# google-research/frame-interpolation

Measured on NVIDIA H100. Metric: interpolated_frames_per_sec_1080p, higher is better.
Workload: dtype f16x2-split (activations/weights as fp16 hi+lo planes; fp32 accumulate)

## Files before the change

frame_interpolation_b200/csrc/film_conv.h:

```cpp
#pragma once
#include <cuda.h>
#include <stdint.h>

#include "film_common.cuh"

namespace film {

constexpr int kMaxSrc = 4;
constexpr int kMaxTaps = 9;
constexpr int kChunk = 64;
constexpr int kTileM = 128;

struct ConvSrc {
  const sp_t* hi;
  const sp_t* lo;
  int C;
  int c_off;
  int nchunk;
  int bswap;
};

struct alignas(64) ConvProblem {
  CUtensorMap tm_a_hi[kMaxSrc];
  CUtensorMap tm_a_lo[kMaxSrc];
// ... 25 lines not shown
  const float* head_b3;
  int crop_y, crop_x, crop_h, crop_w;
  int64_t crop_pitch;
  const float* head_w4;
  const float* head_b4;
  const float* head_vup;
  float* head_res;
  float* head_v;
  int v2_resident;
  int v2_na, v2_nw;
  int v2_grid;
  int v2_part_lo, v2_part_hi;
  sp_t* pool_hi;
  sp_t* pool_lo;
  int pool_C;
  int group;
  int pair;
  int halo;
  int bn;
  int passes;
  int straight;
  int out_lo_skip;
  int pxn;
};

cudaError_t launch_conv_tc(const ConvProblem* d_prob, const ConvProblem& h_prob, cudaStream_t st);
cudaError_t launch_conv_simt(const ConvProblem* d_prob, const ConvProblem& h_prob, cudaStream_t st);
cudaError_t conv_tc_configure();
bool conv3x3_tc_plan(ConvProblem& h_prob, int num_sms);
void conv3x3_tc_pick_tile(int H, int W, int B, int cout, int kc, int passes, int ktot, int epi_mode, int num_sms,
                          int& tile_h, int& tile_w);
cudaError_t launch_conv3x3_tc(const ConvProblem* d_prob, const ConvProblem& h_prob, cudaStream_t st);
cudaError_t conv3x3_tc_configure();
}
```

frame_interpolation_b200/csrc/film_conv3x3_tc.cu:

```cuda
#include <cuda.h>
#include <cuda_runtime.h>
#include <stdint.h>

#include <type_traits>

#include "film_conv.h"
#include "film_tc_ptx.cuh"

namespace film {
namespace {
using namespace tc;

constexpr int kConsumers = 256;
constexpr int kThreads = kConsumers + 128;
__host__ __device__ constexpr int a_plane_bytes(int kc, int th, int tw) { return (th + 2) * tw * kc * 2; }
__host__ __device__ constexpr int a_stage_bytes(int kc, int th, int tw) { return 2 * a_plane_bytes(kc, th, tw); }
constexpr int kHaloW = 10;
__host__ __device__ constexpr int halo_box_bytes(int kc, int th) { return (th + 2) * kHaloW * kc * 2; }
__host__ __device__ constexpr int halo_plane_bytes(int kc, int th) { return (halo_box_bytes(kc, th) + 1023) & ~1023; }
__host__ __device__ constexpr int a_stage_bytes_h(int kc, int th, int tw, int halo, int planes = 2) {
  return planes * (halo ? halo_plane_bytes(kc, th) : a_plane_bytes(kc, th, tw));
}
constexpr int kMaxRing = 8;
constexpr int kSmemLimit = 227 * 1024;
constexpr int kBarBytes = 8 * (4 * kMaxRing + 4);
constexpr int kFixedBytes = kBarBytes + 16 + 512 * 4  + 64  + 1024  + 64;
constexpr int kHeadW3 = 64 * 32 * 4, kHeadMisc = 512;
constexpr int kHeadBytes = kHeadW3 + kHeadMisc;
constexpr int kPxnStageWg = 64 * 64 * 2;
constexpr int kPxnStageBytes = 2 * kPxnStageWg;
inline int epi_scratch_bytes(int epi_mode, int pxn) { return epi_mode == 3 ? kHeadBytes : pxn ? kPxnStageBytes : 0; }

__host__ __device__ inline int w_tap_bytes(int bn, int kc, int planes = 2) { return bn * kc * 2 * planes; }

template <int BN, int KC, bool kPartial, bool kHalo, bool kOne, bool kRes, bool kPxN = false>
__global__ void __launch_bounds__(kThreads, 1) k_conv3x3_tc(const ConvProblem* __restrict__ prob) {
  static_assert(!kPxN || (BN == 64 && KC == 64), "pixels on N: Cout = 64 (one M = 64 weight tile), 64-channel chunks");
  extern __shared__ uint8_t smem_raw[];
  constexpr bool one = kOne;
  const int planes = one ? 1 : 2;
  constexpr int kWPlane = BN * KC * 2;
  const int kWTap = kWPlane * planes;
  const int kTileH = prob->tile_h, kTileW = prob->tile_w;
  constexpr int kHaloTileH = kPxN ? 32 : 16;
  constexpr int kHaloBox = halo_box_bytes(KC, kHaloTileH), kHaloPlane = halo_plane_bytes(KC, kHaloTileH);
  constexpr bool halo = kHalo;
  const int kAPlane = halo ? kHaloPlane : a_plane_bytes(KC, kTileH, kTileW);
  const int kAStage = planes * kAPlane;
  const int kRowStep = kTileW * KC * 2;
  constexpr bool kFused = BN <= 128 && !kPxN;
  constexpr int kAccRegs = kPxN ? 64 : (kFused ? 2 * BN : BN) / 2;
  constexpr int kWgPx = kPxN ? 128 : 64;

  const int NA = prob->v2_na, NW = prob->v2_nw;
  const bool resident = prob->v2_resident != 0;
  const int nsrc = prob->nsrc;
  const int tiles_x = prob->tiles_x, tiles_per_img = prob->tiles_y * prob->tiles_x;
  const int cout = prob->cout;
  const int n_nt = (cout + BN - 1) / BN;
  const int ntiles = prob->B * tiles_per_img * n_nt;
  constexpr int kStageTaps = kHalo ? 9 : 3;
  constexpr bool kPacked = kPartial && kPxN;
  const int part_lo = prob->v2_part_lo, part_hi = prob->v2_part_hi;
  int nab = 0;
// ... 72 lines not shown
      {
        const int nt = tile + w_step;
        int next_sp, nnt;
        decode(nt < nwork ? nt : 0, next_sp, nnt);
        if (nt < nwork && next_sp != sp && next_sp < nsp && elect_one()) {
          int nb, nrem, nty, ntx;
          div_img.divmod(next_sp, nb, nrem);
          div_tx.divmod(nrem, nty, ntx);
          const int ny0 = nty * kTileH, nx0 = ntx * kTileW;
          for (int s = 0; s < nsrc; ++s)
            for (int ch = 0; ch < src_tab[2 * s]; ++ch) {
              const int cc = src_tab[2 * s + 1] + ch * KC;
              tma_prefetch_4d(&prob->tm_a_hi[s], cc, nx0 - 1, ny0 - 1, nb);
              if (!one) tma_prefetch_4d(&prob->tm_a_lo[s], cc, nx0 - 1, ny0 - 1, nb);
              if (!halo) {
                tma_prefetch_4d(&prob->tm_a_hi[s], cc, nx0 + 1, ny0 - 1, nb);
                if (!one) tma_prefetch_4d(&prob->tm_a_lo[s], cc, nx0 + 1, ny0 - 1, nb);
              }
            }
        }
        __syncwarp();
      }
      int kb = 0, ab = 0;
      for (int s = 0; s < nsrc; ++s) {
        const int nchunk = src_tab[2 * s], c_off = src_tab[2 * s + 1];
        const int bs = src_tab[2 * kMaxSrc + s] ? prob->B - 1 - b : b;
        const CUtensorMap* tm_hi = &prob->tm_a_hi[s];
        const CUtensorMap* tm_lo = &prob->tm_a_lo[s];
        for (int ch = 0; ch < nchunk; ++ch) {
          const int nst = halo ? 1 : 3;
          for (int dx = 0; dx < nst; ++dx, ++ab) {
            const int st = ra.stage;
            mbar_wait(tail + 8u * (kMaxRing + st), ra.phase ^ 1u);
            if (elect_one()) {
              const uint32_t sa = a_base + st * kAStage, bar = tail + 8u * st;
              mbar_expect_tx(bar, halo ? (uint32_t)(planes * kHaloBox) : (uint32_t)kAStage);
              tma_load_4d(sa, tm_hi, bar, c_off + ch * KC, x0 + dx - 1, y0 - 1, bs);
              if (!one) tma_load_4d(sa + kAPlane, tm_lo, bar, c_off + ch * KC, x0 + dx - 1, y0 - 1, bs);
            }
            __syncwarp();
            ra.advance(NA);
            if (!resident) {
              const bool packed = kPacked && ab >= part_lo && ab < part_hi;
              const int nblk = packed ? kStageTaps / 3 : kStageTaps;
              for (int t = 0; t < nblk; ++t, ++kb) {
                const int ws = rw.stage;
                mbar_wait(tail + 8u * (3 * kMaxRing + ws), rw.phase ^ 1u);
                if (elect_one()) {
                  const uint32_t sw = w_base + ws * kWTap, bar = tail + 8u * (2 * kMaxRing + ws);
                  mbar_expect_tx(bar, kWTap);
                  if (pair) {
                    const uint32_t hoff = (uint32_t)(rank * (kWPlane / 2));
                    tma_load_2d_mc(sw + hoff, &prob->tm_w_hi_half, bar, kb * KC, n0 + rank * (BN / 2), 3);
                    if (!one) tma_load_2d_mc(sw + kWPlane + hoff, &prob->tm_w_lo_half, bar, kb * KC, n0 + rank * (BN / 2), 3);
                  } else {
                    tma_load_2d(sw, tm_w_hi, bar, kb * KC, n0);
                    if (!one) tma_load_2d(sw + kWPlane, tm_w_lo, bar, kb * KC, n0);
                  }
                }
                __syncwarp();
                rw.advance(NW);
              }
            }
          }
        }
// ... 51 lines not shown
    const uint32_t sbo = kHalo ? kHaloW * kPx : 8 * kPx;
    RingPos ra, rw;
    float acc[kAccRegs];
    for (int tile = w_first; tile < nwork; tile += w_step) {
      int kb = 0;
      int rel_a = -1, rel_w = -1;
      auto retire = [&](int next_a, int next_w) {
        wgmma_commit();
        wgmma_wait<1>();
        if (is_leader) {
          if (rel_a >= 0) mbar_arrive(tail + 8u * (kMaxRing + rel_a));
          if (rel_w >= 0) release_w(rel_w);
        }
        rel_a = next_a;
        rel_w = next_w;
      };
      auto stage = [&](auto ksteps_c, auto tpb_c) {
        constexpr int kSteps = decltype(ksteps_c)::value, kTpb = decltype(tpb_c)::value;
        constexpr int kBlocks = kStageTaps / kTpb;
        const int st = ra.stage;
        mbar_wait(tail + 8u * st, ra.phase);
        const uint32_t sa = a_base + st * kAStage + a_row0;
        const uint32_t lo_off = (uint32_t)(kHalo ? kHaloPlane : kAPlane);
        if constexpr (kRes) {
          const uint64_t a0 = make_desc_sbo<KC>(sa, sbo);
          const uint64_t lo_delta = (uint64_t)(lo_off >> 4);
          const uint64_t row_delta = (uint64_t)(kRowStep >> 4);
          const uint64_t w0 = make_desc_kc<KC>(w_base + kb * kWTapC);
          const uint32_t first = (kb == 0) ? 0u : 1u;
          wgmma_fence();
#pragma unroll
          for (int t = 0; t < kStageTaps; ++t) {
            const uint64_t a_hi = a0 + (kHalo ? (uint64_t)((((t % 3) * kHaloW + t / 3) * kPx) >> 4) : (uint64_t)t * row_delta);
            const uint64_t a_lo = a_hi + lo_delta;
            const uint64_t w_hi = w0 + (uint64_t)(((t / kTpb) * kWTapC + (t % kTpb) * kSteps * 32) >> 4);
            const uint64_t w_lo = w_hi + (uint64_t)(kWPlane >> 4);
#pragma unroll
            for (int k = 0; k < kSteps; ++k) {
              const uint64_t adv = (uint64_t)(k * 32 >> 4);
              const uint32_t accf = (t == 0 && k == 0) ? first : 1u;
              if constexpr (kPxN) {
                wgmma<128>(acc, w_hi + adv, a_hi + adv, accf);
                if constexpr (!kOne) {
                  wgmma<128>(acc, w_lo + adv, a_hi + adv, 1u);
                  wgmma<128>(acc, w_hi + adv, a_lo + adv, 1u);
                }
              } else if constexpr (kOne) {
// ... 63 lines not shown
      };
      using Full = std::integral_constant<int, KC / 16>;
      using One = std::integral_constant<int, 1>;
      if constexpr (kPartial) {
        for (int ab = 0; ab < part_lo; ++ab) stage(Full{}, One{});
        for (int ab = part_lo; ab < part_hi; ++ab) stage(One{}, std::integral_constant<int, kPacked ? 3 : 1>{});
        for (int ab = part_hi; ab < nab; ++ab) stage(Full{}, One{});
      } else {
        for (int ab = 0; ab < nab; ++ab) stage(Full{}, One{});
      }
      wgmma_wait<0>();
      if (is_leader) {
        if (rel_a >= 0) mbar_arrive(tail + 8u * (kMaxRing + rel_a));
        if (rel_w >= 0) release_w(rel_w);
      }
      acc_fence<kAccRegs>(acc);

      int sp, nti, b, rem, ty, tx;
      decode(tile, sp, nti);
      div_img.divmod(sp, b, rem);
      div_tx.divmod(rem, ty, tx);
      const int n0 = nti * BN;
      const bool live = sp < nsp;
      if constexpr (kPxN) {
        const int c0 = 16 * (warp & 3) + (lane >> 2);
        const float bias0 = bias_smem[c0], bias1 = bias_smem[c0 + 8];
#pragma unroll
        for (int i = 0; i < kAccRegs; ++i) {
          const float f = acc[i] + ((i & 2) ? bias1 : bias0);
          acc[i] = act ? leaky(f) : f;
        }
        const int y_wg = ty * kTileH + 16 * wg, x_t = tx * kTileW;
        if (do_pool) {
          const int px = x_t + 2 * q;
#pragma unroll
          for (int j = 0; j < 16; j += 2) {
            const int py = y_wg + j;
            const bool ok = live && (py >> 1) < (out_H >> 1) && (px >> 1) < (out_W >> 1) && !(lane & 4);
            const int64_t ppix = ((int64_t)b * (out_H >> 1) + (py >> 1)) * (out_W >> 1) + (px >> 1);
#pragma unroll
            for (int h = 0; h < 2; ++h) {
              const int i = 4 * j + 2 * h;
              const float v = ((acc[i] + acc[i + 1]) + (acc[i + 4] + acc[i + 5])) * 0.25f;
              const float vn = __shfl_xor_sync(0xffffffffu, v, 4);
              if (ok) {
                uint32_t hi, lo;
// ... 227 lines not shown
  static const int cand[3][2] = {{16, 8}, {8, 16}, {4, 32}};
  const int bn = conv_tc_block_n(cout);
  const int n_nt = (cout + bn - 1) / bn;
  double best = 1e30;
  tile_h = 16;
  tile_w = 8;
  for (auto& c : cand) {
    int res, na, nw;
    if (!ring_depths(kc, c[0], c[1], 0, passes == 1 ? 1 : 2, bn, cout, ktot, epi_mode, 0, res, na, nw)) continue;
    const long tiles = (long)B * ((H + c[0] - 1) / c[0]) * ((W + c[1] - 1) / c[1]) * n_nt;
    const long waves = (tiles + num_sms - 1) / num_sms;
    const double cost = (double)waves * (c[0] + 2.0) / c[0] * (1.0 + 1e-3 * (c[1] / 8));
    if (cost < best) {
      best = cost;
      tile_h = c[0];
      tile_w = c[1];
    }
  }
}

bool conv3x3_tc_plan(ConvProblem& h, int num_sms) {
  const int bn = h.bn;
  const int planes = h.passes == 1 ? 1 : 2;
  const int wtap = w_tap_bytes(bn, h.kchunk, planes);
  const int w_all = (h.ktot / h.kchunk) * wtap;
  const bool can_resident = h.cout <= bn;
  const int kLimit = kSmemLimit - epi_scratch_bytes(h.epi_mode, h.pxn);
  if (h.halo && (h.tile_h != (h.pxn ? 32 : 16) || h.tile_w != 8 ||
                 (can_resident && w_all + 2 * a_stage_bytes_h(h.kchunk, h.tile_h, h.tile_w, 0, planes) + kFixedBytes <= kLimit &&
                  w_all + 2 * a_stage_bytes_h(h.kchunk, h.tile_h, h.tile_w, 1, planes) + kFixedBytes > kLimit)))
    h.halo = 0;
  bool ok = ring_depths(h.kchunk, h.tile_h, h.tile_w, h.halo, planes, bn, h.cout, h.ktot, h.epi_mode, h.pxn,
                        h.v2_resident, h.v2_na, h.v2_nw);
  if (!ok && h.halo) {
    h.halo = 0;
    ok = ring_depths(h.kchunk, h.tile_h, h.tile_w, 0, planes, bn, h.cout, h.ktot, h.epi_mode, h.pxn, h.v2_resident,
                     h.v2_na, h.v2_nw);
  }
  const int nsp = h.B * h.tiles_y * h.tiles_x, n_nt = (h.cout + bn - 1) / bn;
  if (h.pair) {
    const int nwork = (nsp + 1) / 2 * n_nt, nclu = num_sms / 2;
    h.v2_grid = 2 * (nwork < nclu ? nwork : nclu);
  } else {
    h.v2_grid = nsp * n_nt < num_sms ? nsp * n_nt : num_sms;
  }
  return ok;
// ... 22 lines not shown
    if (kPxN && (h.pair || h.tile_h != 32 || h.tile_w != 8 || h.epi_mode != 0)) return cudaErrorInvalidValue;
    const bool partial = h.v2_part_hi > h.v2_part_lo;
    const int idx = (partial ? 8 : 0) | (h.halo ? 4 : 0) | (h.passes == 1 ? 2 : 0) | (h.v2_resident && h.straight ? 1 : 0);
    if (!h.pair) {
      kFn[idx]<<<h.v2_grid, kThreads, smem_bytes_for(h, BN), st>>>(d_prob);
      return cudaGetLastError();
    }
    cudaLaunchConfig_t cfg = {};
    cudaLaunchAttribute attr[1];
    attr[0].id = cudaLaunchAttributeClusterDimension;
    attr[0].val.clusterDim.x = 2;
    attr[0].val.clusterDim.y = 1;
    attr[0].val.clusterDim.z = 1;
    cfg.gridDim = dim3(h.v2_grid);
    cfg.blockDim = dim3(kThreads);
    cfg.dynamicSmemBytes = smem_bytes_for(h, BN);
    cfg.stream = st;
    cfg.attrs = attr;
    cfg.numAttrs = 1;
    return cudaLaunchKernelEx(&cfg, kFn[idx], d_prob);
  }
};

cudaError_t conv3x3_tc_configure() {
  cudaError_t e;
#define FILM_CFG(BN, KC)                        \
  e = Variants<BN, KC>::configure();            \
  if (e != cudaSuccess) return e;
  FILM_CFG(32, 64) FILM_CFG(64, 64) FILM_CFG(128, 64) FILM_CFG(256, 64) FILM_CFG(32, 32) FILM_CFG(64, 32)
#undef FILM_CFG
  e = Variants<64, 64, true>::configure();
  if (e != cudaSuccess) return e;
  return cudaSuccess;
}

cudaError_t launch_conv3x3_tc(const ConvProblem* d_prob, const ConvProblem& h, cudaStream_t st) {
  const int bn = h.bn;
  if (h.kchunk == 32) {
    if (bn == 32) return Variants<32, 32>::launch(d_prob, h, st);
    if (bn == 64) return Variants<64, 32>::launch(d_prob, h, st);
    return cudaErrorInvalidValue;
  }
  switch (bn) {
    case 256: return Variants<256, 64>::launch(d_prob, h, st);
    case 128: return Variants<128, 64>::launch(d_prob, h, st);
    case 64: return h.pxn ? Variants<64, 64, true>::launch(d_prob, h, st) : Variants<64, 64>::launch(d_prob, h, st);
    default: return Variants<32, 64>::launch(d_prob, h, st);
  }
}

}
```

frame_interpolation_b200/csrc/film_engine.cu:

```cuda
#include <cuda.h>
#include <cuda_runtime.h>

#include <algorithm>
#include <cmath>
#include <cstdio>
#include <cstdlib>
#include <cstring>
#include <functional>
#include <map>
#include <memory>
#include <string>
#include <vector>

#include "../../include/film_b200.h"
#include "film_conv.h"
#include "film_kernels.h"
#include "film_pack.h"

namespace film {
int conv_tc_block_n(int cout);

constexpr int kLevels = 7, kFusionLevels = 5, kSpecialized = 3, kSubLevels = 4, kFilters = 64;
static const int kFlowFilters[4] = {32, 64, 128, 256};
static const char* kPredictorNames[4] = {"flow_predictor_0", "flow_predictor_1", "flow_predictor_2",
// ... 33 lines not shown
constexpr uint32_t kDefaultOnepassMask =
    (1u << ST_FE_I0_K23) | (1u << ST_FE_I0_K45) | (1u << ST_FE_I0_K67) |
    (0x1Fu << ST_FLOW_L0) | (0x3Fu << (ST_FUS + 6));

struct Options {
  int conv_impl = 0;
  int use_graph = 1;
  int keep_debug = 0;
  int time_ops = 0;
  int use_lanes = 0;
  int conv3x3_v2 = 1;
  int conv3x3_2cta = 0;
  int conv3x3_halo = 3;
  int conv3x3_pxn = 1;
  int onepass_mask = (int)kDefaultOnepassMask;
  int fe_conv0_tc = 0;
  int fuse_rgb_head = 1;
  int fuse_flow_head = 1;
  int plane_skip = 1;
  int mma_straight = 1;
  int arena_reuse = 1;
  int any_size = 0;
  int tile_overlap = 0;
};

static int as_given(int v) { return v; }
static int as_bool(int v) { return v ? 1 : 0; }
static int clamp_0_2(int v) { return v < 0 ? 0 : (v > 2 ? 2 : v); }
static int non_negative(int v) { return v < 0 ? 0 : v; }
static int stage_bits(int v) { return (int)((uint32_t)v & ((1u << ST_COUNT) - 1u)); }
struct OptionRow {
  const char* name;
  int Options::*field;
  int (*normalise)(int);
  const char* env;
  bool plan_key;
};
static const OptionRow kOptions[] = {
    {"conv_impl", &Options::conv_impl, as_given, nullptr, true},
    {"use_graph", &Options::use_graph, as_given, nullptr, false},
    {"keep_debug", &Options::keep_debug, as_given, nullptr, true},
    {"time_ops", &Options::time_ops, as_given, nullptr, false},
    {"use_lanes", &Options::use_lanes, as_given, nullptr, true},
    {"conv3x3_v2", &Options::conv3x3_v2, as_given, nullptr, true},
    {"conv3x3_2cta", &Options::conv3x3_2cta, as_given, "FILM_2CTA", true},
    {"conv3x3_halo", &Options::conv3x3_halo, as_given, "FILM_HALO", true},
    {"conv3x3_pxn", &Options::conv3x3_pxn, clamp_0_2, nullptr, true},
    {"onepass_mask", &Options::onepass_mask, stage_bits, "FILM_ONEPASS", true},
    {"fe_conv0_tc", &Options::fe_conv0_tc, as_bool, "FILM_FE0_TC", true},
    {"fuse_rgb_head", &Options::fuse_rgb_head, as_bool, "FILM_RGB_FUSE", true},
    {"fuse_flow_head", &Options::fuse_flow_head, clamp_0_2, "FILM_FLOW_HEAD_FUSE", true},
    {"plane_skip", &Options::plane_skip, as_bool, "FILM_PLANE_SKIP", true},
    {"mma_straight", &Options::mma_straight, as_bool, "FILM_STRAIGHT", true},
    {"arena_reuse", &Options::arena_reuse, as_bool, "FILM_ARENA_REUSE", true},
    {"any_size", &Options::any_size, as_bool, nullptr, false},
    {"tile_overlap", &Options::tile_overlap, non_negative, nullptr, false},
};
static const OptionRow& option_row(const char* name) {
  for (const OptionRow& r : kOptions)
    if (!strcmp(r.name, name)) return r;
  throw Error{FILM_ERR_ARG, std::string("unknown option ") + name};
}

#define FILM_CUDA(expr)                                                                       \
  do {                                                                                        \
    cudaError_t e__ = (expr);                                                                 \
    if (e__ != cudaSuccess)                                                                   \
      throw Error{FILM_ERR_CUDA, std::string(#expr) + ": " + cudaGetErrorString(e__)};        \
  } while (0)

struct HostTensor {
  std::vector<int> dims;
  std::vector<float> data;
};
typedef std::map<std::string, HostTensor> WeightMap;

static WeightMap read_weight_file(const char* path) {
  FILE* f = fopen(path, "rb");
  if (!f) throw Error{FILM_ERR_WEIGHTS, std::string("cannot open weight file ") + path};
// ... 70 lines not shown

struct PackedConv {
  sp_t* w_hi = nullptr;
  sp_t* w_lo = nullptr;
  float* bias = nullptr;
  int cout = 0, ktot = 0, cin_ref = 0;
  int kchunk = kChunk;
  std::vector<int> src_chunks;
  std::vector<int> src_ksteps;
  sp_t* pxn_hi = nullptr;
  sp_t* pxn_lo = nullptr;
  int pxn_ktot = 0;
  int ntaps = 0;
  int tap_dy[kMaxTaps], tap_dx[kMaxTaps];
};

struct TapSpec {
  int dy, dx;
  std::vector<std::pair<int, int>> terms;
};

static PackedConv pack_conv(const HostTensor& kernel, const HostTensor& bias,
                            const std::vector<std::vector<int>>& src_maps,
                            const std::vector<TapSpec>& taps, std::vector<void*>& allocs, int chunk = kChunk) {
  const int kw = kernel.dims[1], cin = kernel.dims[2], cout = kernel.dims[3];
  PackedConv pc;
  pc.cout = cout;
  pc.cin_ref = cin;
  pc.kchunk = chunk;
  pc.ntaps = (int)taps.size();
  for (size_t t = 0; t < taps.size(); ++t) {
    pc.tap_dy[t] = taps[t].dy;
    pc.tap_dx[t] = taps[t].dx;
  }
  int ktot = 0;
  for (auto& sm : src_maps) {
    if (sm.size() % chunk) throw Error{FILM_ERR_WEIGHTS, "source channel map not a multiple of the K chunk"};
    pc.src_chunks.push_back((int)sm.size() / chunk);
    int ks = 1;
    for (size_t i = 0; i < sm.size(); ++i)
      if (sm[i] >= 0) ks = std::max(ks, (int)(i % chunk) / 16 + 1);
    pc.src_ksteps.push_back(ks);
    ktot += (int)sm.size() * (int)taps.size();
  }
  pc.ktot = ktot;
  std::vector<uint16_t> hi((size_t)cout * ktot), lo((size_t)cout * ktot);
  int kbase = 0;
// ... 20 lines not shown
    }
  }
  auto upload = [&](const std::vector<uint16_t>& v) {
    sp_t* d;
    FILM_CUDA(cudaMalloc(&d, v.size() * 2));
    allocs.push_back(d);
    FILM_CUDA(cudaMemcpy(d, v.data(), v.size() * 2, cudaMemcpyHostToDevice));
    return d;
  };
  pc.w_hi = upload(hi);
  pc.w_lo = upload(lo);
  pc.pxn_hi = pc.w_hi;
  pc.pxn_lo = pc.w_lo;
  pc.pxn_ktot = ktot;
  std::vector<int> packed;
  for (int ks : pc.src_ksteps) packed.push_back(taps.size() == 9 && chunk == kChunk && ks == 1);
  if (std::count(packed.begin(), packed.end(), 1)) {
    pc.pxn_hi = upload(pack_dx_blocks(hi, cout, ktot, chunk, pc.src_chunks, packed, pc.pxn_ktot));
    pc.pxn_lo = upload(pack_dx_blocks(lo, cout, ktot, chunk, pc.src_chunks, packed, pc.pxn_ktot));
  }
  FILM_CUDA(cudaMalloc(&pc.bias, cout * 4));
  allocs.push_back(pc.bias);
  FILM_CUDA(cudaMemcpy(pc.bias, bias.data.data(), cout * 4, cudaMemcpyHostToDevice));
  return pc;
}

static std::vector<TapSpec> taps_3x3() {
  std::vector<TapSpec> t;
  for (int kx = 0; kx < 3; ++kx)
    for (int ky = 0; ky < 3; ++ky) t.push_back({ky - 1, kx - 1, {{ky, kx}}});
  return t;
}
static std::vector<TapSpec> taps_up2x2(int py, int px) {
  std::vector<TapSpec> t;
  for (int dy = 0; dy <= py; ++dy)
    for (int dx = 0; dx <= px; ++dx) {
      TapSpec s{dy, dx, {}};
      for (int fy = 0; fy < 2; ++fy)
        for (int fx = 0; fx < 2; ++fx)
          if ((py + fy) / 2 == dy && (px + fx) / 2 == dx) s.terms.push_back({fy, fx});
      t.push_back(s);
    }
  return t;
}
static std::vector<int> iota_map(int start, int n, int padded) {
  std::vector<int> m(padded, -1);
  for (int i = 0; i < n; ++i) m[i] = start + i;
  return m;
}
static std::vector<int> side_map(int C) {
  std::vector<int> m(kChunk, -1);
  for (int c = 0; c < 3; ++c) m[c] = c;
  for (int c = 0; c < 3; ++c) m[3 + c] = 3 + C + c;
  m[6] = 6 + 2 * C;
  m[7] = 7 + 2 * C;
  m[8] = 8 + 2 * C;
  m[9] = 9 + 2 * C;
  return m;
}

struct Model {
  std::vector<void*> allocs;
  float *conv0_w = nullptr, *conv0_b = nullptr;
  PackedConv fe[8];
  PackedConv fe0_3x3;
  PackedConv flow[4][3];
  PackedConv flow_c3[4];
  float *flow_w3[4], *flow_b3[4], *flow_w4[4], *flow_b4[4];
  PackedConv fus_up[4][4];
  PackedConv fus_up_2x2[4];
  PackedConv fus_c1[4], fus_c2[4];
  float *rgb_w = nullptr, *rgb_b = nullptr;

  float* upload(const HostTensor& t) {
    float* d;
    FILM_CUDA(cudaMalloc(&d, t.data.size() * 4));
    allocs.push_back(d);
    FILM_CUDA(cudaMemcpy(d, t.data.data(), t.data.size() * 4, cudaMemcpyHostToDevice));
    return d;
  }

  void load(const WeightMap& w) {
    const std::string fe_pre = "feat_net/sub_extractor/cfeat_conv_";
    conv0_w = upload(get_tensor(w, fe_pre + "0/kernel", {3, 3, 3, 64}));
    conv0_b = upload(get_tensor(w, fe_pre + "0/bias", {64}));
    {
      HostTensor k0 = get_tensor(w, fe_pre + "0/kernel", {3, 3, 3, 64});
      k0.dims = {1, 1, 27, 64};
      fe[0] = pack_conv(k0, get_tensor(w, fe_pre + "0/bias", {64}), {iota_map(0, 27, 32)},
                        {TapSpec{0, 0, {{0, 0}}}}, allocs, 32);
      fe0_3x3 = pack_conv(get_tensor(w, fe_pre + "0/kernel", {3, 3, 3, 64}), get_tensor(w, fe_pre + "0/bias", {64}),
                          {iota_map(0, 3, 32)}, taps_3x3(), allocs, 32);
// ... 18 lines not shown
                               get_tensor(w, pre + std::to_string(k) + "/bias", {nf}),
                               {iota_map(0, nf, round_up(nf, kc))}, taps_3x3(), allocs, kc);
      flow_c3[p] = pack_conv(get_tensor(w, pre + "3/kernel", {1, 1, nf, nf / 2}),
                             get_tensor(w, pre + "3/bias", {nf / 2}), {iota_map(0, nf, round_up(nf, kc))},
                             {TapSpec{0, 0, {{0, 0}}}}, allocs, kc);
      flow_w3[p] = upload(get_tensor(w, pre + "3/kernel", {1, 1, nf, nf / 2}));
      flow_b3[p] = upload(get_tensor(w, pre + "3/bias", {nf / 2}));
      flow_w4[p] = upload(get_tensor(w, pre + "4/kernel", {1, 1, nf / 2, 2}));
      flow_b4[p] = upload(get_tensor(w, pre + "4/bias", {2}));
    }
    for (int i = 0; i < kFusionLevels - 1; ++i) {
      const std::string pre = "fusion/level_" + std::to_string(i) + "/conv_";
      const int nf = fusion_filters(i), C = feat_channels(i);
      const bool from_pyr = (i == kFusionLevels - 2);
      const int Cc = feat_channels(i + 1);
      const int coarse_c = from_pyr ? 2 * (3 + Cc) + 4 : fusion_filters(i + 1);
      const HostTensor& k0 = get_tensor(w, pre + "0/kernel", {2, 2, coarse_c, nf});
      const HostTensor& b0 = get_tensor(w, pre + "0/bias", {nf});
      std::vector<std::vector<int>> up_src;
      if (from_pyr)
        up_src = {iota_map(3, Cc, Cc), iota_map(6 + Cc, Cc, Cc), side_map(Cc)};
      else
        up_src = {iota_map(0, coarse_c, coarse_c)};
      for (int py = 0; py < 2; ++py)
        for (int px = 0; px < 2; ++px)
          fus_up[i][py * 2 + px] = pack_conv(k0, b0, up_src, taps_up2x2(py, px), allocs);
      fus_up_2x2[i] = pack_conv(k0, b0, up_src, {{0, 0, {{0, 0}}}, {0, 1, {{0, 1}}}, {1, 0, {{1, 0}}}, {1, 1, {{1, 1}}}},
                                allocs);
      const int a_c = 2 * (3 + C) + 4;
      fus_c1[i] = pack_conv(get_tensor(w, pre + "1/kernel", {3, 3, a_c + nf, nf}),
                            get_tensor(w, pre + "1/bias", {nf}),
                            {iota_map(3, C, C), iota_map(6 + C, C, C), side_map(C),
                             iota_map(a_c, nf, round_up(nf, kChunk))},
                            taps_3x3(), allocs);
      fus_c2[i] = pack_conv(get_tensor(w, pre + "2/kernel", {3, 3, nf, nf}),
                            get_tensor(w, pre + "2/bias", {nf}),
                            {iota_map(0, nf, round_up(nf, kChunk))}, taps_3x3(), allocs);
    }
    rgb_w = upload(get_tensor(w, "fusion/output_conv/kernel", {1, 1, 64, 3}));
    rgb_b = upload(get_tensor(w, "fusion/output_conv/bias", {3}));
  }
  ~Model() {
    for (void* p : allocs) cudaFree(p);
  }
};

typedef CUresult (*EncodeTiledFn)(CUtensorMap*, CUtensorMapDataType, cuuint32_t, void*, const cuuint64_t*,
                                  const cuuint64_t*, const cuuint32_t*, const cuuint32_t*,
                                  CUtensorMapInterleave, CUtensorMapSwizzle, CUtensorMapL2promotion,
// ... 310 lines not shown
  P.mma_flops += (double)cp.passes * 2.0 * (double)cp.B * cp.tiles_y * cp.tiles_x * (cp.tile_h * cp.tile_w) * k_issued *
                 (double)(((pc.cout + bn - 1) / bn) * bn);
  double alg_bytes = 0;
  {
    const double px = (double)cp.B * cp.H * cp.W, planes_in = cp.passes == 1 ? 1.0 : 2.0;
    for (size_t si = 0; si < pc.src_chunks.size(); ++si) alg_bytes += px * pc.src_chunks[si] * pc.kchunk * 2.0 * planes_in;
    if (out) alg_bytes += px * pc.cout * 2.0 * (cp.out_lo_skip ? 1.0 : 2.0);
    if (pool_out) alg_bytes += px / 4.0 * pc.cout * 4.0;
    if (epi_mode == 2) alg_bytes += px * 12.0;
    if (!out && epi_mode != 2) alg_bytes += px * 24.0;
    alg_bytes += (double)pc.cout * ktot * 2.0 * planes_in;
  }
  P.last_conv_bytes = alg_bytes;
  if (no_op) return idx;
  Plan* pp = &P;
  const int impl = o.conv_impl;
  P.add_op(0, tag, [pp, idx, impl, v2](cudaStream_t st) {
    if (impl == 1) return launch_conv_simt(pp->d_probs + idx, pp->h_probs[idx], st);
    return v2 ? launch_conv3x3_tc(pp->d_probs + idx, pp->h_probs[idx], st)
              : launch_conv_tc(pp->d_probs + idx, pp->h_probs[idx], st);
  }, 2.0 * ref_macs_per_px * (double)cp.B * cp.H * cp.W, alg_bytes);
  P.ops.back().form = impl == 1 ? "simt" : !v2 ? "tc" : cp.pxn ? "3x3_pxn" : "3x3";
  return idx;
}

static void padded_size(int h, int w, int align, int& H, int& W, int& off_y, int& off_x) {
  int ph = 0, pw = 0;
  if (align > 0) {
    ph = (h % align) ? align - h % align : 0;
    pw = (w % align) ? align - w % align : 0;
  }
  H = h + ph;
  W = w + pw;
  off_y = ph / 2;
  off_x = pw / 2;
}

static std::unique_ptr<Plan> build_plan(const Model& M, int h, int w, int align, const Options& opt, int num_sms) {
  std::unique_ptr<Plan> pl(new Plan);
  Plan& P = *pl;
  P.opt = opt;
  P.reuse = !opt.keep_debug && !opt.use_lanes && opt.arena_reuse;
  const bool fuse_rgb = opt.conv_impl == 0 && opt.conv3x3_v2 && opt.fuse_rgb_head && !opt.keep_debug;
  P.h = h;
  P.w = w;
  P.num_sms = num_sms;
// ... 258 lines not shown
      std::vector<std::pair<const SplitBuf*, SplitBuf*>> jobs;
      if (i == kFusionLevels - 2) {
        jobs.push_back({wf[i + 1], P.split(2, hh, ww, wf[i + 1]->C)});
        jobs.push_back({side[i + 1], P.split(1, hh, ww, side[i + 1]->C)});
        up_src = {{batch_view(jobs[0].second, 0), 0}, {batch_view(jobs[0].second, 1), 0}, {jobs[1].second, 0}};
      } else {
        jobs.push_back({net, P.split(1, hh, ww, net->C)});
        up_src = {{jobs[0].second, 0}};
      }
      double rbytes = 0;
      for (auto& j : jobs) rbytes += (double)j.second->pixels() * j.second->C * (hi_only ? 4.0 : 8.0);
      P.add_op(2, "fusion_resize@L" + std::to_string(i), [jobs, hi_only](cudaStream_t st) {
        for (auto& j : jobs) {
          const SplitBuf *s = j.first, *d = j.second;
          const cudaError_t e = launch_resize_nearest(s->hi, s->lo, s->C, 0, s->B, s->H, s->W, d->hi, d->lo, d->C, 0, d->H,
                                                      d->W, d->C, hi_only, st);
          if (e != cudaSuccess) return e;
        }
        return cudaSuccess;
      }, 0, rbytes);
      add_conv(P, "fusion_up@L" + std::to_string(i), 4.0 * M.fus_up_2x2[i].cin_ref * nf, M.fus_up_2x2[i], up_src, 0, up, 0,
               ST_FUS + 3 * i, ST_FUS + 3 * i + 1);
      for (auto& j : jobs) P.release(j.second);
    } else if (opt.conv_impl == 0) {
      size_t first = 0;
      for (int py = 0; py < 2; ++py)
        for (int px = 0; px < 2; ++px) {
          const size_t ci = add_conv(P, "", 0, M.fus_up[i][py * 2 + px], up_src, 0, up, 0, ST_FUS + 3 * i, ST_FUS + 3 * i + 1, 2, 2,
                                     py, px, nullptr, true);
          if (py == 0 && px == 0) first = ci;
        }
      P.h_probs[first].group = 4;
      const double up_bytes = 4.0 * P.last_conv_bytes;
      Plan* pq = &P;
      const double fl = 2.0 * 16.0 * M.fus_up[i][0].cin_ref * nf * (double)Hs[i + 1] * Ws[i + 1];
      P.add_op(0, "fusion_up@L" + std::to_string(i), [pq, first](cudaStream_t st) {
        return launch_conv_tc(pq->d_probs + first, pq->h_probs[first], st);
      }, fl, up_bytes);
    } else {
      for (int py = 0; py < 2; ++py)
        for (int px = 0; px < 2; ++px)
          add_conv(P, "fusion_up" + std::to_string(py * 2 + px) + "@L" + std::to_string(i),
                   4.0 * M.fus_up[i][0].cin_ref * nf, M.fus_up[i][py * 2 + px], up_src, 0, up, 0, ST_FUS + 3 * i,
                   ST_FUS + 3 * i + 1, 2, 2, py, px);
    }
    SplitBuf* f1 = P.split(1, hh, ww, cpad);
    SplitBuf* f2 = (fuse_rgb && i == 0) ? nullptr : P.split(1, hh, ww, cpad);
    add_conv(P, "fusion_conv1@L" + std::to_string(i), 9.0 * M.fus_c1[i].cin_ref * nf, M.fus_c1[i],
             {{batch_view(wf[i], 0), 0}, {batch_view(wf[i], 1), 0}, {side[i], 0}, {up, 0}}, 1, f1, 0, ST_FUS + 3 * i + 1,
             ST_FUS + 3 * i + 2);
    if (fuse_rgb && i == 0) {
      const size_t ci = add_conv(P, "fusion_conv2+rgb@L0", 9.0 * nf * nf + 64.0 * 3, M.fus_c2[i], {{f1, 0}}, 1, nullptr, 0,
                                 ST_FUS + 3 * i + 2, ST_NONE, 1, 1, 0, 0, nullptr, false, 2);
      ConvProblem& hp = P.h_probs[ci];
      if (hp.cout != 64 || hp.bn != 64) throw Error{FILM_ERR_UNSUPPORTED, "RGB-head epilogue expects a 64-channel N tile"};
      hp.head_w4 = M.rgb_w;
      hp.head_b4 = M.rgb_b;
      hp.head_v = P.xout;
      hp.crop_y = P.off_y;
      hp.crop_x = P.off_x;
      hp.crop_h = P.h;
// ... 868 lines not shown
```

frame_interpolation_b200/csrc/film_pack.h:

```cpp
#pragma once
#include <stdint.h>

#include <vector>

namespace film {

inline std::vector<uint16_t> pack_dx_blocks(const std::vector<uint16_t>& per_tap, int cout, int ktot, int chunk,
                                            const std::vector<int>& src_chunks, const std::vector<int>& packed,
                                            int& ktot_out) {
  ktot_out = ktot;
  for (size_t s = 0; s < src_chunks.size(); ++s)
    if (packed[s]) ktot_out -= src_chunks[s] * 6 * chunk;
  std::vector<uint16_t> out((size_t)cout * ktot_out, 0);
  for (int n = 0; n < cout; ++n) {
    const uint16_t* src = per_tap.data() + (size_t)n * ktot;
    uint16_t* dst = out.data() + (size_t)n * ktot_out;
    for (size_t s = 0; s < src_chunks.size(); ++s)
      for (int ch = 0; ch < src_chunks[s]; ++ch, src += 9 * chunk) {
        if (!packed[s]) {
          for (int k = 0; k < 9 * chunk; ++k) *dst++ = src[k];
          continue;
        }
        for (int t = 0; t < 9; ++t)
          for (int c = 0; c < 16; ++c) dst[(t / 3) * chunk + (t % 3) * 16 + c] = src[t * chunk + c];
        dst += 3 * chunk;
      }
  }
  return out;
}

}
```

Measured before the change: 26.39.

## Fuse sub-pixel upsampling conv classes into one wide-N persistent wgmma kernel

After: 26.60 (median of 6 runs). No clear change (+0.8%).

```diff
diff --git a/frame_interpolation_b200/csrc/film_conv.h b/frame_interpolation_b200/csrc/film_conv.h
--- a/frame_interpolation_b200/csrc/film_conv.h
+++ b/frame_interpolation_b200/csrc/film_conv.h
@@ -71,6 +71,7 @@
   int straight;
   int out_lo_skip;
   int pxn;
+  int up, up_nf, up_n0, up_kb0;
 };
 
 cudaError_t launch_conv_tc(const ConvProblem* d_prob, const ConvProblem& h_prob, cudaStream_t st);
diff --git a/frame_interpolation_b200/csrc/film_conv3x3_tc.cu b/frame_interpolation_b200/csrc/film_conv3x3_tc.cu
--- a/frame_interpolation_b200/csrc/film_conv3x3_tc.cu
+++ b/frame_interpolation_b200/csrc/film_conv3x3_tc.cu
@@ -5,11 +5,28 @@
 #include <type_traits>
 
 #include "film_conv.h"
+#include "film_pack.h"
 #include "film_tc_ptx.cuh"
 
 namespace film {
 namespace {
 using namespace tc;
+
+constexpr int up_c0(int layout, int u) {
+  int nf = 0, blk = 0, c0 = 0, w = 0;
+  up_layout_block(layout, nf, blk);
+  up_tap_cols(nf, blk, u, c0, w);
+  return c0;
+}
+constexpr int up_w(int layout, int u) {
+  int nf = 0, blk = 0, c0 = 0, w = 0;
+  up_layout_block(layout, nf, blk);
+  up_tap_cols(nf, blk, u, c0, w);
+  return w;
+}
+constexpr int up_last_tap(int layout) { return up_w(layout, 3) ? 3 : up_w(layout, 2) ? 2 : up_w(layout, 1) ? 1 : 0; }
+constexpr int up_slice_w(int layout) { return layout == 1 ? 64 : 128; }
+constexpr int kUpStage = 128;
 
 constexpr int kConsumers = 256;
 constexpr int kThreads = kConsumers + 128;
@@ -33,13 +50,15 @@
 
 __host__ __device__ inline int w_tap_bytes(int bn, int kc, int planes = 2) { return bn * kc * 2 * planes; }
 
-template <int BN, int KC, bool kPartial, bool kHalo, bool kOne, bool kRes, bool kPxN = false>
+template <int BN, int KC, bool kPartial, bool kHalo, bool kOne, bool kRes, bool kPxN = false, int kUp = 0>
 __global__ void __launch_bounds__(kThreads, 1) k_conv3x3_tc(const ConvProblem* __restrict__ prob) {
   static_assert(!kPxN || (BN == 64 && KC == 64), "pixels on N: Cout = 64 (one M = 64 weight tile), 64-channel chunks");
+  static_assert(!kUp || (BN == kUpBlock && KC == 64 && kHalo && !kPartial && !kRes && !kPxN),
+                "sub-pixel upsampling: 256-column N blocks, 64-channel chunks, wide halo, streamed weights");
   extern __shared__ uint8_t smem_raw[];
   constexpr bool one = kOne;
   const int planes = one ? 1 : 2;
-  constexpr int kWPlane = BN * KC * 2;
+  constexpr int kWPlane = (kUp ? kUpStage : BN) * KC * 2;
   const int kWTap = kWPlane * planes;
   const int kTileH = prob->tile_h, kTileW = prob->tile_w;
   constexpr int kHaloTileH = kPxN ? 32 : 16;
@@ -158,6 +177,12 @@
         __syncwarp();
       }
       int kb = 0, ab = 0;
+      int up_slice = 0;
+      if constexpr (kUp > 0) {
+        int unf = 0, ublk = 0;
+        up_layout_block(kUp, unf, ublk);
+        up_slice = prob->up_kb0 + nti * nab * up_slices(unf, ublk);
+      }
       for (int s = 0; s < nsrc; ++s) {
         const int nchunk = src_tab[2 * s], c_off = src_tab[2 * s + 1];
         const int bs = src_tab[2 * kMaxSrc + s] ? prob->B - 1 - b : b;
@@ -176,7 +201,25 @@
             }
             __syncwarp();
             ra.advance(NA);
-            if (!resident) {
+            if constexpr (kUp > 0) {
+              for (int u = 0; u < 4; ++u)
+                for (int p = 0; p < up_w(kUp, u); p += kUpStage) {
+                  const int cols = up_w(kUp, u) - p < kUpStage ? up_w(kUp, u) - p : kUpStage;
+                  const int ws = rw.stage;
+                  mbar_wait(tail + 8u * (3 * kMaxRing + ws), rw.phase ^ 1u);
+                  if (elect_one()) {
+                    const uint32_t sw = w_base + ws * kWTap, bar = tail + 8u * (2 * kMaxRing + ws);
+                    mbar_expect_tx(bar, (uint32_t)(cols * KC * 2 * planes));
+                    for (int j = 0; j < cols / 64; ++j) {
+                      tma_load_2d(sw + j * 64 * KC * 2, tm_w_hi, bar, (up_slice + j) * KC, 0);
+                      if (!one) tma_load_2d(sw + kWPlane + j * 64 * KC * 2, tm_w_lo, bar, (up_slice + j) * KC, 0);
+                    }
+                  }
+                  __syncwarp();
+                  up_slice += cols / 64;
+                  rw.advance(NW);
+                }
+            } else if (!resident) {
               const bool packed = kPacked && ab >= part_lo && ab < part_hi;
               const int nblk = packed ? kStageTaps / 3 : kStageTaps;
               for (int t = 0; t < nblk; ++t, ++kb) {
@@ -274,7 +317,53 @@
         mbar_wait(tail + 8u * st, ra.phase);
         const uint32_t sa = a_base + st * kAStage + a_row0;
         const uint32_t lo_off = (uint32_t)(kHalo ? kHaloPlane : kAPlane);
-        if constexpr (kRes) {
+        if constexpr (kUp > 0) {
+          const uint32_t first = (kb == 0) ? 0u : 1u;
+          auto tap = [&](auto u_c) {
+            constexpr int u = decltype(u_c)::value, c0 = up_c0(kUp, u), w = up_w(kUp, u);
+            if constexpr (w > 0) {
+              static_assert(u > 0 || (c0 == 0 && w == BN), "tap (0, 0) must cover the whole N block");
+              const uint32_t off = (uint32_t)(((u >> 1) + 1) * kHaloW + (u & 1) + 1) * kPx;
+              const uint64_t a_hi = make_desc_sbo<KC>(sa + off, sbo);
+              const uint64_t a_lo = make_desc_sbo<KC>(sa + lo_off + off, sbo);
+              constexpr int S = up_slice_w(kUp), kNst = (w + kUpStage - 1) / kUpStage;
+              static_assert(c0 % S == 0 && w % S == 0 && kUpStage % S == 0, "a tap's range is whole slices of its layout");
+#pragma unroll
+              for (int p = 0; p < kNst; ++p) {
+                const int ws = rw.stage;
+                mbar_wait(tail + 8u * (2 * kMaxRing + ws), rw.phase);
+                const uint32_t sw = w_base + ws * kWTap;
+                const uint64_t w_hi = make_desc_kc<KC>(sw), w_lo = make_desc_kc<KC>(sw + kWPlane);
+                const int cols = w - p * kUpStage < kUpStage ? w - p * kUpStage : kUpStage;
+                wgmma_fence();
+#pragma unroll
+                for (int j = 0; j < cols / S; ++j) {
+                  float* const d = acc + (c0 + p * kUpStage + j * S) / 2;
+                  const uint64_t wj = (uint64_t)((j * S * KC * 2) >> 4);
+#pragma unroll
+                  for (int k = 0; k < KC / 16; ++k) {
+                    const uint64_t adv = (uint64_t)(k * 32 >> 4);
+                    const uint32_t accf = (u == 0 && k == 0) ? first : 1u;
+                    if constexpr (kOne) {
+                      wgmma<S>(d, a_hi + adv, w_hi + wj + adv, accf);
+                    } else {
+                      wgmma<S>(d, a_lo + adv, w_hi + wj + adv, accf);
+                      wgmma<S>(d, a_hi + adv, w_lo + wj + adv, 1u);
+                      wgmma<S>(d, a_hi + adv, w_hi + wj + adv, 1u);
+                    }
+                  }
+                }
+                retire((u == up_last_tap(kUp) && p == kNst - 1) ? st : -1, ws);
+                rw.advance(NW);
+              }
+            }
+          };
+          tap(std::integral_constant<int, 0>{});
+          tap(std::integral_constant<int, 1>{});
+          tap(std::integral_constant<int, 2>{});
+          tap(std::integral_constant<int, 3>{});
+          ++kb;
+        } else if constexpr (kRes) {
           const uint64_t a0 = make_desc_sbo<KC>(sa, sbo);
           const uint64_t lo_delta = (uint64_t)(lo_off >> 4);
           const uint64_t row_delta = (uint64_t)(kRowStep >> 4);
@@ -384,6 +473,43 @@
       div_tx.divmod(rem, ty, tx);
       const int n0 = nti * BN;
       const bool live = sp < nsp;
+      if constexpr (kUp > 0) {
+        const int up_nf = prob->up_nf, up_n0 = prob->up_n0, nf_sh = __ffs(up_nf) - 1;
+        int cy[2], cx[2];
+#pragma unroll
+        for (int h = 0; h < 2; ++h) {
+          const int r = wg * 64 + (warp & 3) * 16 + (lane >> 2) + 8 * h;
+          cy[h] = ty * kTileH + r / kTileW;
+          cx[h] = tx * kTileW + r % kTileW;
+        }
+#pragma unroll
+        for (int j = 0; j < BN / 8; ++j) {
+          const int c = 8 * j + 2 * q, col = up_n0 + n0 + 8 * j;
+          const int g = col >> nf_sh, ch = col - (g << nf_sh) + 2 * q;
+          const int oy = (g == 1 || g == 2) ? 1 : 0, ox = g <= 1 ? 1 : 0;
+#pragma unroll
+          for (int h = 0; h < 2; ++h) {
+            float f0 = acc[4 * j + 2 * h] + bias_smem[n0 + c], f1 = acc[4 * j + 2 * h + 1] + bias_smem[n0 + c + 1];
+            if (act) {
+              f0 = leaky(f0);
+              f1 = leaky(f1);
+            }
+            const int fy = 2 * cy[h] + oy, fx = 2 * cx[h] + ox;
+            if (live && cy[h] < H && cx[h] < W && fy < out_H && fx < out_W) {
+              const int64_t opix = ((int64_t)b * out_H + fy) * out_W + fx;
+              if (lo_skip) {
+                *reinterpret_cast<uint32_t*>(out_hi + opix * out_C + out_c_off + ch) = pack2_hi(f0, f1);
+              } else {
+                uint32_t hi, lo;
+                split_pack2(f0, f1, hi, lo);
+                *reinterpret_cast<uint32_t*>(out_hi + opix * out_C + out_c_off + ch) = hi;
+                *reinterpret_cast<uint32_t*>(out_lo + opix * out_C + out_c_off + ch) = lo;
+              }
+            }
+          }
+        }
+        continue;
+      }
       if constexpr (kPxN) {
         const int c0 = 16 * (warp & 3) + (lane >> 2);
         const float bias0 = bias_smem[c0], bias1 = bias_smem[c0 + 8];
@@ -657,6 +783,16 @@
 bool conv3x3_tc_plan(ConvProblem& h, int num_sms) {
   const int bn = h.bn;
   const int planes = h.passes == 1 ? 1 : 2;
+  if (h.up) {
+    h.halo = 1;
+    h.pair = 0;
+    const bool ok = bn == kUpBlock && h.kchunk == kChunk && h.tile_h == 16 && h.tile_w == 8 &&
+                    ring_depths(h.kchunk, 16, 8, 1, planes, kUpStage, kUpBlock, h.ktot, h.epi_mode, 0, h.v2_resident,
+                                h.v2_na, h.v2_nw);
+    const int items = h.B * h.tiles_y * h.tiles_x * ((h.cout + bn - 1) / bn);
+    h.v2_grid = items < num_sms ? items : num_sms;
+    return ok;
+  }
   const int wtap = w_tap_bytes(bn, h.kchunk, planes);
   const int w_all = (h.ktot / h.kchunk) * wtap;
   const bool can_resident = h.cout <= bn;
@@ -725,8 +861,32 @@
   }
 };
 
+struct UpVariants {
+#define FILM_UP(L) {k_conv3x3_tc<kUpBlock, 64, false, true, false, false, false, L>, \
+                    k_conv3x3_tc<kUpBlock, 64, false, true, true, false, false, L>}
+  static constexpr void (*kFn[7][2])(const ConvProblem*) = {FILM_UP(1), FILM_UP(2), FILM_UP(3), FILM_UP(4),
+                                                             FILM_UP(5), FILM_UP(6), FILM_UP(7)};
+#undef FILM_UP
+  static cudaError_t configure() {
+    for (auto& row : kFn)
+      for (auto fn : row) {
+        const cudaError_t e = cudaFuncSetAttribute(fn, cudaFuncAttributeMaxDynamicSharedMemorySize, kSmemLimit);
+        if (e != cudaSuccess) return e;
+      }
+    return cudaSuccess;
+  }
+  static cudaError_t launch(const ConvProblem* d_prob, const ConvProblem& h, cudaStream_t st) {
+    if (h.up < 1 || h.up > 7 || h.bn != kUpBlock || h.kchunk != kChunk || !h.halo || h.pair || h.v2_resident ||
+        h.v2_na < 2 || h.v2_nw < 2 || h.tile_h != 16 || h.tile_w != 8 || h.epi_mode != 0 || h.v2_part_hi > h.v2_part_lo)
+      return cudaErrorInvalidValue;
+    kFn[h.up - 1][h.passes == 1 ? 1 : 0]<<<h.v2_grid, kThreads, smem_bytes_for(h, kUpStage), st>>>(d_prob);
+    return cudaGetLastError();
+  }
+};
+
 cudaError_t conv3x3_tc_configure() {
-  cudaError_t e;
+  cudaError_t e = UpVariants::configure();
+  if (e != cudaSuccess) return e;
 #define FILM_CFG(BN, KC)                        \
   e = Variants<BN, KC>::configure();            \
   if (e != cudaSuccess) return e;
@@ -739,6 +899,7 @@
 
 cudaError_t launch_conv3x3_tc(const ConvProblem* d_prob, const ConvProblem& h, cudaStream_t st) {
   const int bn = h.bn;
+  if (h.up) return UpVariants::launch(d_prob, h, st);
   if (h.kchunk == 32) {
     if (bn == 32) return Variants<32, 32>::launch(d_prob, h, st);
     if (bn == 64) return Variants<64, 32>::launch(d_prob, h, st);
diff --git a/frame_interpolation_b200/csrc/film_engine.cu b/frame_interpolation_b200/csrc/film_engine.cu
--- a/frame_interpolation_b200/csrc/film_engine.cu
+++ b/frame_interpolation_b200/csrc/film_engine.cu
@@ -79,6 +79,7 @@
   int arena_reuse = 1;
   int any_size = 0;
   int tile_overlap = 0;
+  int conv_up_v2 = 1;
 };
 
 static int as_given(int v) { return v; }
@@ -112,6 +113,7 @@
     {"arena_reuse", &Options::arena_reuse, as_bool, "FILM_ARENA_REUSE", true},
     {"any_size", &Options::any_size, as_bool, nullptr, false},
     {"tile_overlap", &Options::tile_overlap, non_negative, nullptr, false},
+    {"conv_up_v2", &Options::conv_up_v2, clamp_0_2, "FILM_UP_V2", true},
 };
 static const OptionRow& option_row(const char* name) {
   for (const OptionRow& r : kOptions)
@@ -228,7 +230,8 @@
 
 static PackedConv pack_conv(const HostTensor& kernel, const HostTensor& bias,
                             const std::vector<std::vector<int>>& src_maps,
-                            const std::vector<TapSpec>& taps, std::vector<void*>& allocs, int chunk = kChunk) {
+                            const std::vector<TapSpec>& taps, std::vector<void*>& allocs, int chunk = kChunk,
+                            std::vector<uint16_t>* host_hi = nullptr, std::vector<uint16_t>* host_lo = nullptr) {
   const int kw = kernel.dims[1], cin = kernel.dims[2], cout = kernel.dims[3];
   PackedConv pc;
   pc.cout = cout;
@@ -295,7 +298,45 @@
   FILM_CUDA(cudaMalloc(&pc.bias, cout * 4));
   allocs.push_back(pc.bias);
   FILM_CUDA(cudaMemcpy(pc.bias, bias.data.data(), cout * 4, cudaMemcpyHostToDevice));
+  if (host_hi) *host_hi = std::move(hi);
+  if (host_lo) *host_lo = std::move(lo);
   return pc;
+}
+
+struct UpPack {
+  sp_t* w_hi = nullptr;
+  sp_t* w_lo = nullptr;
+  float* bias = nullptr;
+  int nf = 0, kup = 0, nchunk = 0;
+};
+static UpPack pack_up(const PackedConv cls[4], const std::vector<uint16_t> hi[4], const std::vector<uint16_t> lo[4],
+                      const HostTensor& bias, std::vector<void*>& allocs) {
+  UpPack up;
+  up.nf = cls[0].cout;
+  for (int c : cls[0].src_chunks) up.nchunk += c;
+  if (up.nf % 64 || (up.nf < kUpBlock && kUpBlock % up.nf) || (up.nf > kUpBlock && up.nf % kUpBlock))
+    throw Error{FILM_ERR_WEIGHTS, "sub-pixel upsampling conv: unsupported filter count"};
+  std::vector<uint16_t> h[4], l[4];
+  for (int g = 0; g < 4; ++g) {
+    const int pc = up_class_py(g) * 2 + up_class_px(g);
+    h[g] = hi[pc];
+    l[g] = lo[pc];
+  }
+  int kup_lo = 0;
+  const std::vector<uint16_t> ph = pack_up_blocks(h, up.nf, up.nchunk, up.kup), pl = pack_up_blocks(l, up.nf, up.nchunk, kup_lo);
+  auto upload = [&](const void* src, size_t bytes) {
+    void* d;
+    FILM_CUDA(cudaMalloc(&d, bytes));
+    allocs.push_back(d);
+    FILM_CUDA(cudaMemcpy(d, src, bytes, cudaMemcpyHostToDevice));
+    return d;
+  };
+  up.w_hi = (sp_t*)upload(ph.data(), ph.size() * 2);
+  up.w_lo = (sp_t*)upload(pl.data(), pl.size() * 2);
+  std::vector<float> b(4 * up.nf);
+  for (int n = 0; n < 4 * up.nf; ++n) b[n] = bias.data[n % up.nf];
+  up.bias = (float*)upload(b.data(), b.size() * 4);
+  return up;
 }
 
 static std::vector<TapSpec> taps_3x3() {
@@ -341,6 +382,7 @@
   PackedConv flow_c3[4];
   float *flow_w3[4], *flow_b3[4], *flow_w4[4], *flow_b4[4];
   PackedConv fus_up[4][4];
+  UpPack fus_up_sp[4];
   PackedConv fus_up_2x2[4];
   PackedConv fus_c1[4], fus_c2[4];
   float *rgb_w = nullptr, *rgb_b = nullptr;
@@ -405,9 +447,12 @@
         up_src = {iota_map(3, Cc, Cc), iota_map(6 + Cc, Cc, Cc), side_map(Cc)};
       else
         up_src = {iota_map(0, coarse_c, coarse_c)};
+      std::vector<uint16_t> cls_hi[4], cls_lo[4];
       for (int py = 0; py < 2; ++py)
         for (int px = 0; px < 2; ++px)
-          fus_up[i][py * 2 + px] = pack_conv(k0, b0, up_src, taps_up2x2(py, px), allocs);
+          fus_up[i][py * 2 + px] = pack_conv(k0, b0, up_src, taps_up2x2(py, px), allocs, kChunk, &cls_hi[py * 2 + px],
+                                             &cls_lo[py * 2 + px]);
+      fus_up_sp[i] = pack_up(fus_up[i], cls_hi, cls_lo, b0, allocs);
       fus_up_2x2[i] = pack_conv(k0, b0, up_src, {{0, 0, {{0, 0}}}, {0, 1, {{0, 1}}}, {1, 0, {{1, 0}}}, {1, 1, {{1, 1}}}},
                                 allocs);
       const int a_c = 2 * (3 + C) + 4;
@@ -764,6 +809,97 @@
   }, 2.0 * ref_macs_per_px * (double)cp.B * cp.H * cp.W, alg_bytes);
   P.ops.back().form = impl == 1 ? "simt" : !v2 ? "tc" : cp.pxn ? "3x3_pxn" : "3x3";
   return idx;
+}
+
+static void add_up_conv(Plan& P, const std::string& tag, const UpPack& up, const PackedConv& cls0,
+                        const std::vector<SrcRef>& sources, const SplitBuf* out, int stage, int consumer,
+                        double ref_flops, double alg_bytes) {
+  const int nf = up.nf, nblk = 4 * nf / kUpBlock;
+  if ((int)sources.size() != (int)cls0.src_chunks.size()) throw Error{FILM_ERR_WEIGHTS, "source count mismatch"};
+  std::vector<size_t> parts;
+  int slice = 0;
+  for (int blk = 0; blk < nblk;) {
+    const int layout = up_layout(nf, blk);
+    int n = 1;
+    while (blk + n < nblk && up_layout(nf, blk + n) == layout) ++n;
+    ConvProblem cp;
+    memset(&cp, 0, sizeof(cp));
+    cp.passes = P.onepass(stage) ? 1 : 3;
+    cp.out_lo_skip = P.hi_only(consumer) ? 1 : 0;
+    const SplitBuf* s0 = sources[0].buf;
+    cp.nsrc = (int)sources.size();
+    cp.B = s0->B;
+    cp.H = s0->H;
+    cp.W = s0->W;
+    cp.kchunk = kChunk;
+    cp.tile_h = 16;
+    cp.tile_w = 8;
+    cp.tiles_y = (cp.H + cp.tile_h - 1) / cp.tile_h;
+    cp.tiles_x = (cp.W + cp.tile_w - 1) / cp.tile_w;
+    for (int s = 0; s < cp.nsrc; ++s) {
+      const SplitBuf* b = sources[s].buf;
+      if (b->B != cp.B || b->H != cp.H || b->W != cp.W) throw Error{FILM_ERR_ARG, "conv source grid mismatch"};
+      cp.src[s].hi = b->hi;
+      cp.src[s].lo = b->lo;
+      cp.src[s].C = b->C;
+      cp.src[s].c_off = sources[s].c_off;
+      cp.src[s].nchunk = cls0.src_chunks[s];
+      cp.src[s].bswap = sources[s].bswap;
+      if (sources[s].c_off + cls0.src_chunks[s] * kChunk > b->C) throw Error{FILM_ERR_ARG, "conv source channel overrun"};
+      make_act_map(&cp.tm_a_hi[s], b->hi, b->B, b->H, b->W, b->C, cp.tile_h + 2, cp.tile_w + 2, kChunk);
+      make_act_map(&cp.tm_a_lo[s], b->lo, b->B, b->H, b->W, b->C, cp.tile_h + 2, cp.tile_w + 2, kChunk);
+    }
+    cp.ntaps = 4;
+    for (int u = 0; u < 4; ++u) {
+      cp.tap_dy[u] = u >> 1;
+      cp.tap_dx[u] = u & 1;
+    }
+    cp.ktot = up.nchunk * kChunk * up_slices(nf, blk);
+    cp.w_hi = up.w_hi;
+    cp.w_lo = up.w_lo;
+    cp.bias = up.bias + blk * kUpBlock;
+    cp.cout = n * kUpBlock;
+    cp.act = 0;
+    cp.out_hi = out->hi;
+    cp.out_lo = out->lo;
+    cp.out_C = out->C;
+    cp.out_H = out->H;
+    cp.out_W = out->W;
+    cp.out_sy = cp.out_sx = 2;
+    cp.group = 1;
+    cp.bn = kUpBlock;
+    make_w_map(&cp.tm_w_hi, up.w_hi, 64, up.kup, 64, kChunk);
+    make_w_map(&cp.tm_w_lo, up.w_lo, 64, up.kup, 64, kChunk);
+    cp.up = layout;
+    cp.up_nf = nf;
+    cp.up_n0 = blk * kUpBlock;
+    cp.up_kb0 = slice;
+    if (out->B != cp.B || out->C < nf || out->H > 2 * cp.H || out->W > 2 * cp.W)
+      throw Error{FILM_ERR_ARG, "conv destination mismatch"};
+    if (!conv3x3_tc_plan(cp, P.num_sms))
+      throw Error{FILM_ERR_UNSUPPORTED, "persistent 3x3 conv: shared-memory rings do not fit (" + tag + ")"};
+    parts.push_back(P.h_probs.size());
+    P.h_probs.push_back(cp);
+    int cols = 0;
+    for (int u = 0; u < 4; ++u) {
+      int c0 = 0, w = 0;
+      up_tap_cols(nf, blk, u, c0, w);
+      cols += w;
+    }
+    P.mma_flops += (double)cp.passes * 2.0 * (double)cp.B * cp.tiles_y * cp.tiles_x * (cp.tile_h * cp.tile_w) *
+                   (double)up.nchunk * kChunk * cols * n;
+    slice += n * up.nchunk * up_slices(nf, blk);
+    blk += n;
+  }
+  Plan* pp = &P;
+  P.add_op(0, tag, [pp, parts](cudaStream_t st) {
+    for (size_t idx : parts) {
+      const cudaError_t e = launch_conv3x3_tc(pp->d_probs + idx, pp->h_probs[idx], st);
+      if (e != cudaSuccess) return e;
+    }
+    return cudaSuccess;
+  }, ref_flops, alg_bytes);
+  P.ops.back().form = "3x3_up";
 }
 
 static void padded_size(int h, int w, int align, int& H, int& W, int& off_y, int& off_x) {
@@ -1068,6 +1204,14 @@
       add_conv(P, "fusion_up@L" + std::to_string(i), 4.0 * M.fus_up_2x2[i].cin_ref * nf, M.fus_up_2x2[i], up_src, 0, up, 0,
                ST_FUS + 3 * i, ST_FUS + 3 * i + 1);
       for (auto& j : jobs) P.release(j.second);
+    } else if (opt.conv_impl == 0 && opt.conv3x3_v2 && (opt.conv_up_v2 >= 2 || (opt.conv_up_v2 == 1 && (nf == 64 || nf >= 512)))) {
+      const PackedConv& c11 = M.fus_up[i][3];
+      const double px = (double)Hs[i + 1] * Ws[i + 1], planes = P.onepass(ST_FUS + 3 * i) ? 1.0 : 2.0;
+      double cls_bytes = px * nf * 2.0 * (P.hi_only(ST_FUS + 3 * i + 1) ? 1.0 : 2.0) + (double)nf * c11.ktot * 2.0 * planes;
+      for (int c : c11.src_chunks) cls_bytes += px * c * kChunk * 2.0 * planes;
+      const double fl = 2.0 * 16.0 * M.fus_up[i][0].cin_ref * nf * (double)Hs[i + 1] * Ws[i + 1];
+      add_up_conv(P, "fusion_up@L" + std::to_string(i), M.fus_up_sp[i], c11, up_src, up, ST_FUS + 3 * i,
+                  ST_FUS + 3 * i + 1, fl, 4.0 * cls_bytes);
     } else if (opt.conv_impl == 0) {
       size_t first = 0;
       for (int py = 0; py < 2; ++py)
@@ -1083,6 +1227,7 @@
       P.add_op(0, "fusion_up@L" + std::to_string(i), [pq, first](cudaStream_t st) {
         return launch_conv_tc(pq->d_probs + first, pq->h_probs[first], st);
       }, fl, up_bytes);
+      P.ops.back().form = "tc";
     } else {
       for (int py = 0; py < 2; ++py)
         for (int px = 0; px < 2; ++px)
diff --git a/frame_interpolation_b200/csrc/film_pack.h b/frame_interpolation_b200/csrc/film_pack.h
--- a/frame_interpolation_b200/csrc/film_pack.h
+++ b/frame_interpolation_b200/csrc/film_pack.h
@@ -29,4 +29,61 @@
   return out;
 }
 
+constexpr int up_class_py(int g) { return (g == 1 || g == 2) ? 1 : 0; }
+constexpr int up_class_px(int g) { return g <= 1 ? 1 : 0; }
+constexpr int kUpBlock = 256;
+
+constexpr void up_tap_cols(int nf, int blk, int u, int& c0, int& w) {
+  int lo = 1 << 30, hi = -1;
+  for (int g = 0; g < 4; ++g) {
+    if ((u >> 1) > up_class_py(g) || (u & 1) > up_class_px(g)) continue;
+    const int a = g * nf > blk * kUpBlock ? g * nf : blk * kUpBlock;
+    const int b = (g + 1) * nf < (blk + 1) * kUpBlock ? (g + 1) * nf : (blk + 1) * kUpBlock;
+    if (a < b) {
+      lo = a < lo ? a : lo;
+      hi = b > hi ? b : hi;
+    }
+  }
+  c0 = hi > lo ? lo - blk * kUpBlock : 0;
+  w = hi > lo ? hi - lo : 0;
 }
+constexpr int up_layout(int nf, int blk) { return nf == 64 ? 1 : nf == 128 ? 2 + blk : 4 + blk * kUpBlock / nf; }
+constexpr void up_layout_block(int layout, int& nf, int& blk) {
+  nf = layout == 1 ? 64 : layout <= 3 ? 128 : 256;
+  blk = layout == 1 ? 0 : layout <= 3 ? layout - 2 : layout - 4;
+}
+constexpr int up_slices(int nf, int blk) {
+  int n = 0;
+  for (int u = 0; u < 4; ++u) {
+    int c0 = 0, w = 0;
+    up_tap_cols(nf, blk, u, c0, w);
+    n += w / 64;
+  }
+  return n;
+}
+
+inline std::vector<uint16_t> pack_up_blocks(const std::vector<uint16_t> cls[4], int nf, int nchunk, int& kup) {
+  const int nblk = 4 * nf / kUpBlock;
+  int slices = 0;
+  for (int blk = 0; blk < nblk; ++blk) slices += nchunk * up_slices(nf, blk);
+  kup = 64 * slices;
+  std::vector<uint16_t> out((size_t)64 * kup, 0);
+  int s = 0;
+  for (int blk = 0; blk < nblk; ++blk)
+    for (int ch = 0; ch < nchunk; ++ch)
+      for (int u = 0; u < 4; ++u) {
+        int c0 = 0, w = 0;
+        up_tap_cols(nf, blk, u, c0, w);
+        for (int j = 0; j < w / 64; ++j, ++s)
+          for (int r = 0; r < 64; ++r) {
+            const int col = blk * kUpBlock + c0 + 64 * j + r, g = col / nf, n = col % nf;
+            const int px1 = up_class_px(g) + 1, ntaps = (up_class_py(g) + 1) * px1;
+            const int t = (u >> 1) * px1 + (u & 1);
+            const uint16_t* src = cls[g].data() + (size_t)n * nchunk * ntaps * 64 + ((size_t)ch * ntaps + t) * 64;
+            for (int c = 0; c < 64; ++c) out[(size_t)r * kup + (size_t)s * 64 + c] = src[c];
+          }
+      }
+  return out;
+}
+
+}
```
